# armando-palacio/opticomlib

Hardware: AMD Instinct MI355X
Metric: SSFM sample*steps/sec, 2^20-sample dual-pol fiber (higher is better)
Workload: dtype c64

## Files before the change

### opticomlib_amd/csrc/ssfm_host.hip

```cpp
#include <hip/hip_runtime.h>

#include <algorithm>
#include <memory>
#include <cmath>
#include <cstdarg>
#include <cstddef>
#include <cstdio>
#include <cstdlib>
#include <chrono>
#include <cstring>
#include <atomic>
#include <condition_variable>
#include <functional>
#include <mutex>
#include <new>
#include <string>
#include <thread>
#include <type_traits>
#include <vector>

#include "ssfm_amd.h"
#include "ssfm_common.hpp"
#include "ssfm_kernels.hpp"
#include "ssfm_launch.hpp"
// ... 687 lines not shown
            lanes_from_pool = true;
            ++g_lane_pairs_reused;
        }
        if (!lane_stream[0]) HIP_TRY(hipStreamCreateWithPriority(lane_stream[0].out(), hipStreamNonBlocking, prio_hi));
        stream = lane_stream[0];
        for (Event* e : {&ev0, &ev1}) HIP_TRY(hipEventCreate(e->out()));
        if (const char* e = std::getenv("SSFM_LANE_THREADS")) lane_threads = std::atoi(e) != 0;
        HIP_TRY(hipEventCreateWithFlags(fork_ev.out(), hipEventDisableTiming));
        for (int g = 1; g < nlanes; ++g) {
            if (!(lanes_from_pool && g == 1)) HIP_TRY(hipStreamCreateWithPriority(lane_stream[g].out(), hipStreamNonBlocking, prio_hi));
            HIP_TRY(hipEventCreateWithFlags(lane_ev[g].out(), hipEventDisableTiming));
        }
        lanes_active = nlanes;
        return SSFM_OK;
    }
    int make_tables() {
        HIP_TRY(F_own.reserve(cb * n * batch));
        HIP_TRY(P_own.reserve(sizeof(T) * n * batch));
        F = F_own; P = P_own;
        Y = F;
        if (u16) { HIP_TRY(Y_own.reserve(cb * n * batch)); Y = Y_own; }
        if (u16 || sizeof(T) == 8) {
            const long long nA = (long long)(N1 / E) * N2, nB = (long long)E * N2;
            HIP_TRY(twA.reserve(cb * nA));
            HIP_TRY(twB.reserve(cb * nB));
            const int C_ = cols_per_tile<T>();
            hipLaunchKernelGGL(k_make_tw_tiles<T>, dim3((unsigned)((nA + 255) / 256)), dim3(256), 0, stream, twA.get(), N1 / E, 1ll, N2, C_, (long long)n, (int)u16, N2 / Ef);
            hipLaunchKernelGGL(k_make_tw_tiles<T>, dim3((unsigned)((nB + 255) / 256)), dim3(256), 0, stream, twB.get(), E, (long long)(N1 / E), N2, C_, (long long)n, (int)u16, N2 / Ef);
        } else {
            HIP_TRY(twN.reserve(cb * n));
            hipLaunchKernelGGL(k_make_twN<T>, dim3((unsigned)((n + 255) / 256)), dim3(256), 0, stream, twN.get(), N1, N2, cols_per_tile<T>(), E, (int)u16, N2 / Ef);
        }
        if (int rc = make_line_table(&tw1, N1, E)) return rc;
        if (int rc = make_line_table(&tw2, N2, Ef)) return rc;
        HIP_TRY(dnat.reserve(cb * n_full));
        HIP_TRY(dperm.reserve(cb * n));
        return SSFM_OK;
    }
    int make_split_extras() {
        HIP_TRY(Fnat.reserve(cb * n_full * batch_full));
        HIP_TRY(hipMemsetAsync(Fnat, 0, cb * n_full * batch_full, stream));
        HIP_TRY(split_twA.reserve(sizeof(double2) * (size_t)split_R * N1));
        HIP_TRY(split_twB.reserve(sizeof(double2) * (size_t)split_R * N2));
        const long long nt = (long long)split_R * (N1 + N2);
        hipLaunchKernelGGL(k_make_split_twiddles, dim3((unsigned)((nt + 255) / 256)), dim3(256), 0, stream, split_twA.get(), split_twB.get(), N1, N2, split_R);
        HIP_TRY(hipGetLastError());
        return SSFM_OK;
    }
    int make_engine_extras() {
        if (Ef_fly != Ef) {
            if (int rc = make_line_table(&tw2_fly, N2, Ef_fly)) return rc;
            HIP_TRY(dperm_fly.reserve(cb * n));
        }
        if (const char* e = std::getenv("SSFM_ADAPT_FUSED")) fused_ok = std::atoi(e) != 0;
        if (const char* e = std::getenv("SSFM_MEDIUM")) medium_ok = std::atoi(e) != 0;
        if (const char* e = std::getenv("SSFM_MEDIUM_ADAPT")) medium_adapt_ok = std::atoi(e) != 0;
        if (const char* e = std::getenv("SSFM_MEDIUM_SPLIT")) medium_split_ok = std::atoi(e) != 0;
        if (const char* e = std::getenv("SSFM_FUSED_PATIENCE_TICKS")) medium_patience = std::atoll(e);
        if (const char* e = std::getenv("SSFM_PHASE_TABLE")) phase_tables = std::atoi(e) != 0;
        if (const char* e = std::getenv("SSFM_FORCE_FLY")) force_fly = std::atoi(e) != 0;
        if (sizeof(T) == 4 && medium_shape(N1, N2) && (medium_ok || medium_adapt_ok)) (void)pick_xcc();
        if (small) {
            if (int rc = make_line_table(&tw_small, (int)n, small_points<T>((int)n))) return rc;
            HIP_TRY(dsmall.reserve(cb * n));
        }
        HIP_TRY(st.reserve(sizeof(AdaptState<T>)));
        HIP_TRY(hipMemsetAsync(P, 0, sizeof(T) * n * batch, stream));
        HIP_TRY(hipGetLastError());
        HIP_TRY(hipStreamSynchronize(stream));
        return SSFM_OK;
    }
    int rate_lanes_at_creation() {
        for (Event* e : {&lane_e0, &lane_e1, &run_e0, &run_e1}) HIP_TRY(hipEventCreate(e->out()));
        HIP_TRY(hipMemsetAsync(F, 0, cb * n * batch, stream));
        if (Y != F) HIP_TRY(hipMemsetAsync(Y, 0, cb * n * batch, stream));
        HIP_TRY(hipMemsetAsync(dperm, 0, cb * n, stream));
        if (dperm_fly) HIP_TRY(hipMemsetAsync(dperm_fly, 0, cb * n, stream));
        bool replaced = false;
        if (lanes_from_pool && nlanes == 2) lanes_ok = true;
        else {
            ++g_lane_ratings;
            if (int rc = rate_and_replace_lanes(F, Y, P, &replaced)) return rc;
        }
        if (!lanes_ok) lane_strikes = 1;
// ... 124 lines not shown
        else lane_suspect = 0;
        return SSFM_OK;
    }
    int heal_lanes() {
        ++lane_heals;
        HIP_TRY(hipStreamSynchronize(stream));
        const size_t cb = sizeof(cx<T>) * (size_t)n * batch;
        DeviceBuffer<cx<T>> Fx_own, Yx_own;
        DeviceBuffer<T> Px_own;
        if (Fx_own.reserve(cb) != hipSuccess) { (void)hipGetLastError(); return SSFM_OK; }
        if (Y != F && Yx_own.reserve(cb) != hipSuccess) { (void)hipGetLastError(); return SSFM_OK; }
        if (Px_own.reserve(sizeof(T) * (size_t)n * batch) != hipSuccess) { (void)hipGetLastError(); return SSFM_OK; }
        cx<T>* const Fx = Fx_own; cx<T>* const Yx = Y != F ? Yx_own.get() : Fx; T* const Px = Px_own;
        (void)hipMemsetAsync(Fx, 0, cb, stream);
        if (Yx != Fx) (void)hipMemsetAsync(Yx, 0, cb, stream);
        (void)hipMemsetAsync(Px, 0, sizeof(T) * (size_t)n * batch, stream);
        const float seen = lane_pair_us;
        bool replaced = false;
        const int rc = rate_and_replace_lanes(Fx, Yx, Px, &replaced);
        (void)hipStreamSynchronize(stream);
        if (rc != SSFM_OK) return rc;
        if (replaced) ++lanes_remade;
        if (lanes_ok) {
            lane_strikes = 0;
            if (!replaced) lane_pair_us = lane_last_us;
            else if (seen > 0.f && seen < lane_pair_us) lane_pair_us = seen;
        } else if (++lane_strikes >= 2) {
            lanes_active = 1;
            lanes_dropped = 1;
        }
        return SSFM_OK;
    }

    int make_line_table(DeviceBuffer<cx<T>>* out, int L, int E) {
        const int M = fft_nstages(L, E);
        const int total = fft_tw_entries(L, E, (int)sizeof(T));
        std::vector<cx<T>> tab((size_t)(total > 0 ? total : 1));
        for (int S = 1; S < M; ++S) {
            const int R = fft_radix(L, S, E), NB = E / R, KU = fft_tw_ku(L, S, E), off = fft_tw_offset(L, S, E, (int)sizeof(T));
            for (int i = 0; i < NB; ++i)
                for (int u = 1; u < R; ++u)
                    for (int ku = 0; ku < KU; ++ku) {
                        const int q = fft_tw_exponent(L, E, S, i, u, ku) % L;
                        const double ang = -2.0 * 3.14159265358979323846 * (double)q / (double)L;
                        cx<T> w; w.x = (T)std::cos(ang); w.y = (T)std::sin(ang);
                        if (q == 0) { w.x = (T)1; w.y = (T)0; }
                        if (4 * q == L) { w.x = (T)0; w.y = (T)-1; }
                        if (2 * q == L) { w.x = (T)-1; w.y = (T)0; }
                        if (4 * q == 3 * L) { w.x = (T)0; w.y = (T)1; }
                        tab[(size_t)off + (size_t)fft_tw_index(L, S, E, (int)sizeof(T), i * (R - 1) + (u - 1), ku)] = w;
                    }
        }
        HIP_TRY(out->reserve(sizeof(cx<T>) * tab.size()));
        HIP_TRY(hipMemcpy(out->get(), tab.data(), sizeof(cx<T>) * tab.size(), hipMemcpyHostToDevice));
        return SSFM_OK;
    }

#if SSFM_TRACE
    DeviceBuffer<unsigned long long> trace_buf;
    int trace_cap = 0; std::atomic<int> trace_next{0};
    std::vector<int> trace_kind;
    int trace_begin(int launches) {
        if (!std::getenv("SSFM_TRACE_FILE")) return SSFM_OK;
        if (trace_cap < launches) {
            HIP_TRY(trace_buf.reserve(sizeof(unsigned long long) * 1024 * launches));
            trace_cap = launches;
        }
        HIP_TRY(hipMemset(trace_buf, 0, sizeof(unsigned long long) * 1024 * launches));
        trace_next = 0;
        trace_kind.assign(launches, 0);
        return SSFM_OK;
    }
    template <typename A> void trace_tag(A& a, int kind, int lane) {
        a.trace = nullptr; a.trace_slot = 0;
        if (trace_buf) { const int slot = trace_next.fetch_add(1); if (slot < trace_cap) { a.trace = trace_buf; a.trace_slot = slot; trace_kind[slot] = kind * 16 + lane; } }
    }
    int trace_dump() {
        const char* path = std::getenv("SSFM_TRACE_FILE");
        if (!path || !trace_buf) return SSFM_OK;
        HIP_TRY(hipStreamSynchronize(stream));
        const int nt = std::min((int)trace_next, trace_cap);
        std::vector<unsigned long long> raw(1024 * (size_t)nt), h(4 * (size_t)nt);
        HIP_TRY(hipMemcpy(raw.data(), trace_buf, sizeof(unsigned long long) * raw.size(), hipMemcpyDeviceToHost));
        for (int i = 0; i < nt; ++i) {
            unsigned long long fs = ~0ull, ls = 0, fe = ~0ull, le = 0;
// ... 1816 lines not shown
```

### opticomlib_amd/csrc/ssfm_kernels.hpp

```cpp
#pragma once
#include "ssfm_route.hpp"
#include "wgfft.hpp"

#ifndef SSFM_ABLATE
#define SSFM_ABLATE 0
#endif
#define SSFM_ABL_NO_TWN ((SSFM_ABLATE & 1) != 0)
#define SSFM_ABL_NO_P ((SSFM_ABLATE & 2) != 0)
#define SSFM_ABL_NO_TAB ((SSFM_ABLATE & 4) != 0)
#define SSFM_ABL_NO_FFT ((SSFM_ABLATE & 8) != 0)
#define SSFM_ABL_NO_NL ((SSFM_ABLATE & 16) != 0)

template <typename T, bool U16> __host__ __device__ constexpr bool stream_policy() { return U16; }
template <typename T, bool U16> __host__ __device__ constexpr bool twn_compute() { return U16 || sizeof(T) == 8; }

#ifndef SSFM_TRACE
#define SSFM_TRACE 0
#endif
#if SSFM_TRACE
#define SSFM_TRACE_ARGS unsigned long long* trace; int trace_slot;
#define SSFM_TRACE_BEGIN(a)                                                                     \
    if ((a).trace && threadIdx.x == 0) {                                                        \
        unsigned hw_, xc_;                                                                      \
        asm volatile("s_getreg_b32 %0, hwreg(HW_REG_HW_ID)" : "=s"(hw_));                       \
// ... 1142 lines not shown
        const double e = flat ? e0 : exp_acc<double>(m[t].x * h);
        m[t] = mk<double>((e * cs) * inv_n, (e * sn) * inv_n);
    }
}

template <typename T, int N2, int ROWS, int E, int MODE, bool U16, bool PK = false, bool H = false>
__device__ __forceinline__ void freq_body(const FreqArgs<T>& a, const unsigned bid) {
    static_assert(!H || (sizeof(T) == 8 && !U16 && !PK && MODE == FM_TABLE), "H (see time_body): the plain layout of a complex128 plan, a table of complex numbers");
    constexpr int Q = N2 / E;
    extern __shared__ __attribute__((aligned(16))) unsigned char smem_raw[];
    cx<T>* lds = reinterpret_cast<cx<T>*>(smem_raw);

    T h = a.h;
    constexpr bool FLY = MODE == FM_FLY || MODE == FM_FLY_IM;
    SSFM_TRACE_BEGIN(a);
    const int tid = threadIdx.x;
    const int j = tid % Q;
    const int rr = tid / Q;
    int kgrp, brow;
    xcd_unit_row(bid, a.N1 / ROWS, a.rows, kgrp, brow);
    const int k1 = kgrp * ROWS + rr;
    const long long row = (long long)brow * a.N1 + k1;
    cx<T>* __restrict__ Frow = a.F + row * N2;
    const cx<T>* __restrict__ trow = a.tab + (MODE == FM_TABLE_ROWS ? row : (long long)k1) * N2;
    using RI = RowIdx<row_pad_shift(E)>;
    const RI idx{rr * row_lds_elems(N2, E)};

    cx<T> v[E];
    cx<T> m[E];
    LineTw<T, N2, E> tw;
    SSFM_STAMP(0);
    typedef T u4_t __attribute__((ext_vector_type(4)));
    constexpr bool EARLY_PHASE = MODE == FM_PHASE;
    TwStaged<T, N2, E, ROWS * N2 / E> tws;
    line_twiddles_prefetch<T, N2, E, ROWS * N2 / E>(tws, a.tw2, tid);
    unsigned pu[E];
    double pt[sizeof(T) == 8 ? E : 1];
    auto load_phases = [&]() {
        if constexpr (sizeof(T) == 8) {
            typedef double d2_t __attribute__((ext_vector_type(2)));
            const d2_t* __restrict__ P2 = reinterpret_cast<const d2_t*>(reinterpret_cast<const double*>(a.tab) + (long long)k1 * N2) + j;
#pragma unroll
            for (int g = 0; g < E / 2; ++g) {
                const d2_t q = P2[g * Q];
                pt[2 * g] = q.x; pt[2 * g + 1] = q.y;
            }
        } else {
        typedef unsigned u32x4 __attribute__((ext_vector_type(4)));
        const u32x4* __restrict__ P4 = reinterpret_cast<const u32x4*>(reinterpret_cast<const unsigned*>(a.tab) + (long long)k1 * N2) + j;
#pragma unroll
        for (int g = 0; g < E / 4; ++g) {
            u32x4 q;
            if (SSFM_ABL_NO_TAB) q = 0x12345678u; else q = P4[g * Q];
            pu[4 * g] = q.x; pu[4 * g + 1] = q.y; pu[4 * g + 2] = q.z; pu[4 * g + 3] = q.w;
        }
        }
    };
    auto phase_factors = [&]() {
#pragma unroll
        for (int t = 0; t < E; ++t) {
            if constexpr (sizeof(T) == 8) m[t] = phase64_factor(pt[t], a.amp);
            else m[t] = phase32_factor(pu[t], a.amp);
        }
    };
    constexpr bool EARLY_FLY = FLY;
    auto load_table = [&]() {
        if constexpr (MODE == FM_FLY_IM) {
// ... 16 lines not shown
            m[2 * g] = mk<T>(q.x, q.y);
            m[2 * g + 1] = mk<T>(q.z, q.w);
        }
    };
    if constexpr (EARLY_PHASE) load_phases();
    if constexpr (EARLY_FLY) load_table();
    constexpr bool INV_ONLY = MODE == FM_INV_ONLY;
    if (U16 && (!INV_ONLY || a.u16 == 2)) {
        if constexpr (PK && sizeof(T) == 4) {
            const __amdgpu_buffer_rsrc_t rs = __builtin_amdgcn_make_buffer_rsrc((void*)Frow, 0, N2 * (int)sizeof(cx<T>), 0x00020000);
#pragma unroll
            for (int g = 0; g < E / 2; ++g) {
                const u32x4_t q = load16_sc1(rs, (g * Q + j) * 16);
                v[2 * g] = mk<T>(__uint_as_float(q.x), __uint_as_float(q.y));
                v[2 * g + 1] = mk<T>(__uint_as_float(q.z), __uint_as_float(q.w));
            }
        } else {
#pragma unroll
        for (int g = 0; g < E / 2; ++g) {
            const u4_t q = stream_load<true>(reinterpret_cast<const u4_t*>(Frow) + g * Q + j);
            v[2 * g] = mk<T>(q.x, q.y);
            v[2 * g + 1] = mk<T>(q.z, q.w);
        }
        }
    } else if constexpr (H) {
        const cx<float>* __restrict__ F32 = reinterpret_cast<const cx<float>*>(a.F) + row * N2;
#pragma unroll
        for (int t = 0; t < E; ++t) { const cx<float> q = F32[j + t * Q]; v[t] = mk<T>((T)q.x, (T)q.y); }
    } else {
#pragma unroll
        for (int t = 0; t < E; ++t) v[t] = Frow[j + t * Q];
    }
    cx<T>* ldsT = lds + (fft_nstages(N2, E) > 1 ? ROWS * row_lds_elems(N2, E) : 0);
    line_twiddles_issue_regs<T, N2, E>(tw, j, a.tw2);
    if constexpr (MODE == FM_TABLE || MODE == FM_TABLE_ROWS) load_table();
    if ((FLY || MODE == FM_FWD_ONLY || MODE == FM_INV_ONLY) && a.st != nullptr) {
        const StepState<T> S = a.st->cur[a.step & 1];
        if (S.done || a.st->error != 0u) return;
        h = S.h;
    }
    SSFM_STAMP(1);
#if SSFM_STAMPS
    asm volatile("s_waitcnt vmcnt(0)" ::: "memory");
    SSFM_STAMP(2);
#endif
    line_twiddles_commit<T, N2, E, ROWS * N2 / E>(tws, ldsT, tid);
    auto fly = [&]() {
        T ph[E];
#pragma unroll
        for (int t = 0; t < E; ++t) ph[t] = m[t].y * h;
        bool flat = true;
#pragma unroll
        for (int t = 1; t < E; ++t) flat = flat && (m[t].x == m[0].x);
        const T e0 = exp_acc<T>(m[0].x * h);
        fly_factors<E>(m, ph, flat, e0, h, a.inv_n);
    };
    if constexpr (EARLY_PHASE) {
        phase_factors();
        __builtin_amdgcn_sched_barrier(0);
    }
    if constexpr (EARLY_FLY) {
        fly();
        __builtin_amdgcn_sched_barrier(0);
    }
    if (fft_tw_lds_entries(N2, E) > 0) __syncthreads();
    line_twiddles_fetch<T, N2, E>(tw, j, ldsT);
    if (!SSFM_ABL_NO_FFT && !INV_ONLY) fft_line<T, N2, E, -1, 0, RI>(v, lds, 0, j, idx, tw);
    if (MODE == FM_FWD_ONLY) {
        if (U16 && a.u16 == 2) {
#pragma unroll
            for (int g = 0; g < E / 2; ++g) {
                u4_t q;
                q.x = v[2 * g].x; q.y = v[2 * g].y; q.z = v[2 * g + 1].x; q.w = v[2 * g + 1].y;
                pass_store<PK>(reinterpret_cast<u4_t*>(Frow) + g * Q + j, q);
            }
            return;
        }
#pragma unroll
        for (int t = 0; t < E; ++t) pass_store<PK>(&Frow[j + t * Q], v[t]);
        return;
    }
    SSFM_STAMP(3);
    if constexpr (!INV_ONLY) {
#pragma unroll
    for (int t = 0; t < E; ++t) v[t] = cmul(v[t], m[t]);
    }
    SSFM_STAMP(4);
    if (!SSFM_ABL_NO_FFT) fft_line<T, N2, E, +1, (fft_nstages(N2, E) == 1 ? 0 : 1), RI>(v, lds, 0, j, idx, tw);
    SSFM_STAMP(5);
    if (U16) {
#pragma unroll
        for (int g = 0; g < E / 2; ++g) {
            u4_t q;
            q.x = v[2 * g].x; q.y = v[2 * g].y; q.z = v[2 * g + 1].x; q.w = v[2 * g + 1].y;
            pass_store<PK>(reinterpret_cast<u4_t*>(Frow) + g * Q + j, q);
        }
    } else if constexpr (H) {
        cx<float>* __restrict__ F32 = reinterpret_cast<cx<float>*>(a.F) + row * N2;
#pragma unroll
// ... 12 lines not shown
    SSFM_TRACE_END(a);
}

template <typename T, int N2, int ROWS, int E, int MODE, bool U16 = false>
__global__ SSFM_KERNEL_BOUNDS(ROWS * N2 / E, sizeof(T), E) void k_freq(cx<T>* F, const cx<T>* tab, const cx<T>* tw2, const AdaptState<T>* st, T h, T amp, T inv_n, int step, int N1,
                                                                     int rows, int u16
#if SSFM_TRACE
                                                                     , unsigned long long* trace, int trace_slot
#endif
                                                                     ) {
    FreqArgs<T> a;
    a.F = F; a.tab = tab; a.tw2 = tw2; a.st = st; a.h = h; a.amp = amp; a.inv_n = inv_n; a.step = step; a.N1 = N1; a.rows = rows; a.u16 = u16;
#if SSFM_TRACE
    a.trace = trace; a.trace_slot = trace_slot;
#endif
    freq_body<T, N2, ROWS, E, MODE, U16, false>(a, blockIdx.x);
}
template <typename T, int N2, int ROWS, int E, int MODE>
__global__ SSFM_KERNEL_BOUNDS(ROWS * N2 / E, sizeof(T), E) void k_freq_h(cx<T>* F, const cx<T>* tab, const cx<T>* tw2, const AdaptState<T>* st, T h, T amp, T inv_n, int step, int N1,
                                                                       int rows, int u16, const int* done
#if SSFM_TRACE
                                                                       , unsigned long long* trace, int trace_slot
#endif
                                                                       ) {
    if (done != nullptr && *done) return;
    FreqArgs<T> a;
    a.F = F; a.tab = tab; a.tw2 = tw2; a.st = st; a.h = h; a.amp = amp; a.inv_n = inv_n; a.step = step; a.N1 = N1; a.rows = rows; a.u16 = u16;
#if SSFM_TRACE
    a.trace = trace; a.trace_slot = trace_slot;
#endif
    freq_body<T, N2, ROWS, E, MODE, false, false, true>(a, blockIdx.x);
}
template <typename T, int N2, int ROWS, int E, int MODE, bool U16 = false>
__global__ __launch_bounds__(ROWS * N2 / E) void k_freq_half(cx<T>* F, const cx<T>* tab, const cx<T>* tw2, const AdaptState<T>* st, T h, T amp, T inv_n, int step, int N1,
                                                            int rows, int u16
#if SSFM_TRACE
                                                            , unsigned long long* trace, int trace_slot
#endif
                                                            ) {
    static_assert(MODE == FM_FWD_ONLY || MODE == FM_INV_ONLY, "k_freq_half: the transform-only modes");
    FreqArgs<T> a;
    a.F = F; a.tab = tab; a.tw2 = tw2; a.st = st; a.h = h; a.amp = amp; a.inv_n = inv_n; a.step = step; a.N1 = N1; a.rows = rows; a.u16 = u16;
#if SSFM_TRACE
    a.trace = trace; a.trace_slot = trace_slot;
#endif
    freq_body<T, N2, ROWS, E, MODE, U16, false>(a, blockIdx.x);
}
#if SSFM_TRACE
#define SSFM_FREQ_KERNEL_ARGS(a) (a).F, (a).tab, (a).tw2, (a).st, (a).h, (a).amp, (a).inv_n, (a).step, (a).N1, (a).rows, (a).u16, (a).trace, (a).trace_slot
#else
#define SSFM_FREQ_KERNEL_ARGS(a) (a).F, (a).tab, (a).tw2, (a).st, (a).h, (a).amp, (a).inv_n, (a).step, (a).N1, (a).rows, (a).u16
#endif

constexpr int kSmallTabs = 4;
template <typename T> struct MediumArgs {
    cx<T>* F;
    cx<T>* Y;
    T* P;
    const cx<T>* twA;
    const cx<T>* twB;
    const cx<T>* tw1;
    const cx<T>* tw2;
    const cx<T>* tab[kSmallTabs];
    T amp[kSmallTabs];
    const T* hs;
    const unsigned char* which;
    unsigned long long* bar;
// ... 958 lines not shown
```

### opticomlib_amd/csrc/ssfm_launch.hpp

```cpp
#pragma once
#include <hip/hip_runtime.h>

#include <cstddef>

#include "ssfm_kernels.hpp"

namespace ssfm {
template <typename T> constexpr size_t col_pass_lds(int N1, int C, int E) {
    return ((fft_nstages(N1, E) > 1 ? (size_t)N1 * C : 0) + (size_t)E * C + (size_t)fft_tw_lds_entries(N1, E)) * sizeof(cx<T>);
}
template <typename T> constexpr size_t row_pass_lds(int N, int E, int ROWS, size_t extra = 0) {
    return ((fft_nstages(N, E) > 1 ? (size_t)ROWS * row_lds_elems(N, E) : 0) + (size_t)fft_tw_lds_entries(N, E) + extra) * sizeof(cx<T>);
}

template <auto Kernel, size_t LDS, typename... Args>
hipError_t launch_kernel(dim3 grid, dim3 block, hipStream_t s, const Args&... args) {
    if constexpr (LDS > 48 * 1024) {
        static const hipError_t raised = hipFuncSetAttribute(reinterpret_cast<const void*>(Kernel), hipFuncAttributeMaxDynamicSharedMemorySize, (int)LDS);
        if (raised != hipSuccess) return raised;
    }
    hipLaunchKernelGGL(Kernel, grid, block, LDS, s, args...);
    return hipGetLastError();
}
}
```

### opticomlib_amd/csrc/wgfft.hpp

```cpp
#pragma once
#include <hip/hip_runtime.h>

#ifndef SSFM_STAMPS
#define SSFM_STAMPS 0
#endif
#if SSFM_STAMPS
extern __device__ unsigned long long* g_stamp_buf;
#define SSFM_STAMP(i)                                                                         \
    do {                                                                                      \
        __builtin_amdgcn_sched_barrier(0);                                                    \
        if (threadIdx.x == 0) {                                                               \
            unsigned long long t_;                                                            \
            asm volatile("s_memtime %0\n\ts_waitcnt lgkmcnt(0)" : "=s"(t_)::"memory");         \
            g_stamp_buf[blockIdx.x * 16 + (i)] = t_;                                          \
        }                                                                                     \
        __builtin_amdgcn_sched_barrier(0);                                                    \
    } while (0)
#else
#define SSFM_STAMP(i) do { } while (0)
#endif


namespace ssfm {

typedef float  cf32 __attribute__((ext_vector_type(2)));
typedef double cf64 __attribute__((ext_vector_type(2)));
template <typename T> struct cx_of;
template <> struct cx_of<float>  { using type = cf32; };
template <> struct cx_of<double> { using type = cf64; };
template <typename T> using cx = typename cx_of<T>::type;
template <typename C> struct real_of;
template <> struct real_of<cf32> { using type = float; };
template <> struct real_of<cf64> { using type = double; };

// ... 98 lines not shown
        x[0] = cadd(e0, o0); x[4] = csub(e0, o0);
        x[1] = cadd(e1, o1); x[5] = csub(e1, o1);
        x[2] = add_rot<DIR>(e2, o2); x[6] = sub_rot<DIR>(e2, o2);
        x[3] = cadd(e3, o3); x[7] = csub(e3, o3);
    }
};
template <> struct Dft<16> {
    template <int DIR, typename C> static __device__ __forceinline__ void run(C* x) {
        using T = typename real_of<C>::type;
        using K = RadixConst<T>;
#pragma unroll
        for (int b = 0; b < 4; ++b) dft4<DIR>(x[b], x[b + 4], x[b + 8], x[b + 12]);
        x[1 + 4]  = cmuld<DIR>(x[1 + 4], mk<T>(K::cA, -K::sA));
        x[1 + 8]  = mul_w8_1<DIR, 1>(x[1 + 8]);
        x[1 + 12] = cmuld<DIR>(x[1 + 12], mk<T>(K::sB, -K::cB));
        x[2 + 4]  = mul_w8_1<DIR, 0>(x[2 + 4]);
        x[2 + 8]  = rot90<DIR>(x[2 + 8]);
        x[2 + 12] = mul_w8_3<DIR, 1>(x[2 + 12]);
        x[3 + 4]  = cmuld<DIR>(x[3 + 4], mk<T>(K::sB, -K::cB));
        x[3 + 8]  = mul_w8_3<DIR, 0>(x[3 + 8]);
        x[3 + 12] = cmuld<DIR>(x[3 + 12], mk<T>(-K::cB, K::sB));
        C y[16];
#pragma unroll
        for (int q = 0; q < 4; ++q) {
            C a = x[4 * q], b = x[4 * q + 1], c = x[4 * q + 2], d = x[4 * q + 3];
            dft4<DIR>(a, b, c, d);
            y[q] = a; y[q + 4] = b; y[q + 8] = c; y[q + 12] = d;
        }
#pragma unroll
        for (int i = 0; i < 16; ++i) x[i] = y[i];
    }
};

__host__ __device__ constexpr int ilog2(int v) { return v <= 1 ? 0 : 1 + ilog2(v >> 1); }
__host__ __device__ constexpr int fft_nstages(int L, int E) {
    return E == 16 ? (L <= 16 ? 1 : (L <= 256 ? 2 : (L <= 4096 ? 3 : 4))) : (ilog2(L) + 2) / 3;
}
__host__ __device__ constexpr int fft_radix(int L, int s, int E) {
    return E == 16 ? (L == 16   ? 16
                    : L == 32   ? (s == 0 ? 8 : 4)
                    : L == 64   ? 8
                    : L == 128  ? (s == 0 ? 16 : 8)
                    : L == 256  ? 16
                    : L == 512  ? 8
                    : L == 1024 ? (s == 0 ? 16 : 8)
                    : L == 2048 ? (s <= 1 ? 16 : 8)
                    : L == 4096 ? 16
                    :             (s <= 2 ? 16 : 2))
                   : (s < ilog2(L) / 3 ? 8 : (1 << (ilog2(L) % 3)));
}
__host__ __device__ constexpr int fft_ls(int L, int s, int E) {
    return s == 0 ? 1 : fft_ls(L, s - 1, E) * fft_radix(L, s - 1, E);
}

template <typename T, int E, int L = 0> __host__ __device__ constexpr bool tw_lazy() {
    return sizeof(T) == 8 && E == 16;
}

template <typename T, int L, int E, bool LAZY = tw_lazy<T, E, L>()> struct LineTw {
    static constexpr int M = fft_nstages(L, E);
    cx<T> w[M > 1 ? M - 1 : 1][E - 1];
};
template <typename T, int L, int E> struct LineTw<T, L, E, true> {
    static constexpr int M = fft_nstages(L, E);
    const cx<T>* g[M > 1 ? M - 1 : 1];
    const cx<T>* l[M > 1 ? M - 1 : 1];
};
__host__ __device__ constexpr int fft_tw_slots_of(int L, int S, int E) { return (E / fft_radix(L, S, E)) * (fft_radix(L, S, E) - 1); }
__host__ __device__ constexpr int fft_tw_ku(int L, int S, int E) { return fft_ls(L, S, E) < L / E ? fft_ls(L, S, E) : L / E; }
__host__ __device__ constexpr bool fft_tw_via_lds(int L, int S, int E) { return fft_tw_slots_of(L, S, E) * fft_tw_ku(L, S, E) <= 512; }
__host__ __device__ constexpr bool fft_tw_paired(int L, int S, int E, int ts) {
    return ts == 4 && !fft_tw_via_lds(L, S, E);
}
__host__ __device__ constexpr int fft_tw_stage_entries(int L, int S, int E, int ts) {
    return fft_tw_paired(L, S, E, ts) ? ((fft_tw_slots_of(L, S, E) + 1) / 2) * 2 * fft_tw_ku(L, S, E)
                                      : ((fft_tw_slots_of(L, S, E) * fft_tw_ku(L, S, E) + 1) / 2) * 2;
}
__host__ __device__ constexpr int fft_tw_offset(int L, int S, int E, int ts) {
    return S <= 1 ? 0 : fft_tw_offset(L, S - 1, E, ts) + fft_tw_stage_entries(L, S - 1, E, ts);
}
__host__ __device__ constexpr int fft_tw_entries(int L, int E, int ts) { return fft_tw_offset(L, fft_nstages(L, E), E, ts); }
__host__ __device__ constexpr int fft_tw_index(int L, int S, int E, int ts, int slot, int ku) {
    return fft_tw_paired(L, S, E, ts) ? ((slot >> 1) * fft_tw_ku(L, S, E) + ku) * 2 + (slot & 1) : slot * fft_tw_ku(L, S, E) + ku;
}
__host__ __device__ constexpr int fft_tw_lds_offset(int L, int S, int E) {
    return S <= 1 ? 0 : fft_tw_lds_offset(L, S - 1, E) + (fft_tw_via_lds(L, S - 1, E) ? fft_tw_slots_of(L, S - 1, E) * fft_tw_ku(L, S - 1, E) : 0);
}
__host__ __device__ constexpr int fft_tw_lds_entries(int L, int E) { return fft_tw_lds_offset(L, fft_nstages(L, E), E); }
__host__ __device__ constexpr int fft_tw_exponent(int L, int E, int S, int i, int u, int ku) {
    return ((ku + i * (L / E)) & (fft_ls(L, S, E) - 1)) * u * (L / (fft_ls(L, S, E) * fft_radix(L, S, E)));
}

template <typename T, int L, int E, int S>
__device__ __forceinline__ void tw_stage_issue(LineTw<T, L, E>& tw, const int j, const cx<T>* __restrict__ tab, cx<T>* ldsT,
                                               const int tid, const int nthreads) {
    constexpr int SLOTS = fft_tw_slots_of(L, S, E);
    constexpr int KU = fft_tw_ku(L, S, E);
    constexpr int OFF = fft_tw_offset(L, S, E, (int)sizeof(T));
    if constexpr (fft_tw_paired(L, S, E, (int)sizeof(T))) {
        typedef T w4_t __attribute__((ext_vector_type(4)));
        const w4_t* __restrict__ p4 = reinterpret_cast<const w4_t*>(tab + OFF) + (j & (KU - 1));
#pragma unroll
        for (int pr = 0; pr < (SLOTS + 1) / 2; ++pr) {
            const w4_t q = p4[pr * KU];
            tw.w[S - 1][2 * pr] = mk<T>(q.x, q.y);
            if (2 * pr + 1 < SLOTS) tw.w[S - 1][2 * pr + 1] = mk<T>(q.z, q.w);
        }
    } else if constexpr (fft_tw_via_lds(L, S, E)) {
        constexpr int LOFF = fft_tw_lds_offset(L, S, E);
        for (int e = tid; e < SLOTS * KU; e += nthreads) ldsT[LOFF + e] = tab[OFF + e];
    } else if constexpr (tw_lazy<T, E, L>()) {
        tw.g[S - 1] = tab + OFF + (j & (KU - 1));
    } else {
#pragma unroll
        for (int sl = 0; sl < SLOTS; ++sl) tw.w[S - 1][sl] = tab[OFF + sl * KU + (j & (KU - 1))];
    }
}
template <typename T, int L, int E, int S>
__device__ __forceinline__ void tw_stage_fetch(LineTw<T, L, E>& tw, const int j, const cx<T>* ldsT) {
    if constexpr (fft_tw_via_lds(L, S, E)) {
        constexpr int SLOTS = fft_tw_slots_of(L, S, E);
        constexpr int KU = fft_tw_ku(L, S, E);
        constexpr int LOFF = fft_tw_lds_offset(L, S, E);
        if constexpr (tw_lazy<T, E, L>()) {
            tw.l[S - 1] = ldsT + LOFF + (j & (KU - 1));
        } else {
#pragma unroll
            for (int sl = 0; sl < SLOTS; ++sl) tw.w[S - 1][sl] = ldsT[LOFF + sl * KU + (j & (KU - 1))];
        }
    }
}
template <typename T, int L, int E, int S>
__device__ __forceinline__ cx<T> tw_get(const LineTw<T, L, E>& tw, const int slot) {
    if constexpr (tw_lazy<T, E, L>()) {
        constexpr int KU = fft_tw_ku(L, S, E);
        if constexpr (fft_tw_via_lds(L, S, E)) return tw.l[S - 1][slot * KU];
        else return tw.g[S - 1][slot * KU];
    } else {
        return tw.w[S - 1][slot];
    }
}
template <typename T, int L, int E>
__device__ __forceinline__ void line_twiddles_issue(LineTw<T, L, E>& tw, const int j, const cx<T>* __restrict__ tab, cx<T>* ldsT,
                                                    const int tid, const int nthreads) {
    constexpr int M = fft_nstages(L, E);
    if constexpr (M > 1) tw_stage_issue<T, L, E, 1>(tw, j, tab, ldsT, tid, nthreads);
    if constexpr (M > 2) tw_stage_issue<T, L, E, 2>(tw, j, tab, ldsT, tid, nthreads);
    if constexpr (M > 3) tw_stage_issue<T, L, E, 3>(tw, j, tab, ldsT, tid, nthreads);
}
__host__ __device__ constexpr int fft_tw_prefetch_count(int L, int E, int NT, int S = 1) {
    return S >= fft_nstages(L, E) ? 0
         : (fft_tw_via_lds(L, S, E) ? (fft_tw_slots_of(L, S, E) * fft_tw_ku(L, S, E) + NT - 1) / NT : 0) + fft_tw_prefetch_count(L, E, NT, S + 1);
}
template <typename T, int L, int E, int NT> struct TwStaged {
    static constexpr int PF = fft_tw_prefetch_count(L, E, NT);
    cx<T> r[PF > 0 ? PF : 1];
};
template <typename T, int L, int E, int NT, int S>
__device__ __forceinline__ void tw_stage_prefetch(TwStaged<T, L, E, NT>& p, int& k, const cx<T>* __restrict__ tab, const int tid) {
    if constexpr (fft_tw_via_lds(L, S, E)) {
        constexpr int NS = fft_tw_slots_of(L, S, E) * fft_tw_ku(L, S, E), OFF = fft_tw_offset(L, S, E, (int)sizeof(T));
#pragma unroll
        for (int i = 0; i * NT < NS; ++i) {
            const int e = tid + i * NT;
            p.r[k++] = e < NS ? tab[OFF + e] : mk<T>((T)0, (T)0);
        }
    }
}
template <typename T, int L, int E, int NT, int S>
__device__ __forceinline__ void tw_stage_commit(const TwStaged<T, L, E, NT>& p, int& k, cx<T>* ldsT, const int tid) {
    if constexpr (fft_tw_via_lds(L, S, E)) {
        constexpr int NS = fft_tw_slots_of(L, S, E) * fft_tw_ku(L, S, E), LOFF = fft_tw_lds_offset(L, S, E);
#pragma unroll
        for (int i = 0; i * NT < NS; ++i) {
            const int e = tid + i * NT;
            if (e < NS) ldsT[LOFF + e] = p.r[k];
            ++k;
        }
    }
}
template <typename T, int L, int E, int NT>
__device__ __forceinline__ void line_twiddles_prefetch(TwStaged<T, L, E, NT>& p, const cx<T>* __restrict__ tab, const int tid) {
    constexpr int M = fft_nstages(L, E);
    int k = 0;
    if constexpr (M > 1) tw_stage_prefetch<T, L, E, NT, 1>(p, k, tab, tid);
    if constexpr (M > 2) tw_stage_prefetch<T, L, E, NT, 2>(p, k, tab, tid);
    if constexpr (M > 3) tw_stage_prefetch<T, L, E, NT, 3>(p, k, tab, tid);
}
template <typename T, int L, int E, int NT>
__device__ __forceinline__ void line_twiddles_commit(const TwStaged<T, L, E, NT>& p, cx<T>* ldsT, const int tid) {
    constexpr int M = fft_nstages(L, E);
    int k = 0;
    if constexpr (M > 1) tw_stage_commit<T, L, E, NT, 1>(p, k, ldsT, tid);
    if constexpr (M > 2) tw_stage_commit<T, L, E, NT, 2>(p, k, ldsT, tid);
    if constexpr (M > 3) tw_stage_commit<T, L, E, NT, 3>(p, k, ldsT, tid);
}
template <typename T, int L, int E>
__device__ __forceinline__ void line_twiddles_issue_regs(LineTw<T, L, E>& tw, const int j, const cx<T>* __restrict__ tab) {
    constexpr int M = fft_nstages(L, E);
    if constexpr (M > 1 && !fft_tw_via_lds(L, 1, E)) tw_stage_issue<T, L, E, 1>(tw, j, tab, nullptr, 0, 1);
    if constexpr (M > 2 && !fft_tw_via_lds(L, 2, E)) tw_stage_issue<T, L, E, 2>(tw, j, tab, nullptr, 0, 1);
    if constexpr (M > 3 && !fft_tw_via_lds(L, 3, E)) tw_stage_issue<T, L, E, 3>(tw, j, tab, nullptr, 0, 1);
}
template <typename T, int L, int E>
__device__ __forceinline__ void line_twiddles_fetch(LineTw<T, L, E>& tw, const int j, const cx<T>* ldsT) {
    constexpr int M = fft_nstages(L, E);
    if constexpr (M > 1) tw_stage_fetch<T, L, E, 1>(tw, j, ldsT);
    if constexpr (M > 2) tw_stage_fetch<T, L, E, 2>(tw, j, ldsT);
    if constexpr (M > 3) tw_stage_fetch<T, L, E, 3>(tw, j, ldsT);
}

template <typename T, int L, int E, int DIR, int S, int XP, typename IDX>
__device__ __forceinline__ void fft_stage(cx<T> (&v)[E], cx<T>* lds, const int BUF, const int j, const IDX& idx,
                                          const LineTw<T, L, E>& tw) {
    constexpr int M  = fft_nstages(L, E);
    constexpr int R  = fft_radix(L, S, E);
    constexpr int NB = E / R;
    constexpr int Q  = L / E;
    constexpr int LS = fft_ls(L, S, E);

#ifdef SSFM_STAMP_FFT
    if (DIR < 0) SSFM_STAMP_FFT(7 + 3 * S);
#endif
    if constexpr (S > 0) {
        const cx<T>* src = lds + ((XP + S - 1) & 1) * BUF;
#pragma unroll
        for (int i = 0; i < NB; ++i) {
            const int jb = j + i * Q;
#pragma unroll
            for (int u = 0; u < R; ++u) v[i + u * NB] = src[idx(jb + u * (L / R))];
        }
#pragma unroll
        for (int i = 0; i < NB; ++i) {
#pragma unroll
            for (int u = 1; u < R; ++u)
                v[i + u * NB] = cmuld<DIR>(v[i + u * NB], tw_get<T, L, E, S>(tw, i * (R - 1) + (u - 1)));
        }
    }
#ifdef SSFM_STAMP_FFT
    if (DIR < 0) SSFM_STAMP_FFT(8 + 3 * S);
#endif
#pragma unroll
// ... 49 lines not shown
```

Baseline: 68.34 billion.

## Replace large per-stage row-FFT twiddle tables with a compact quarter-wave table in LDS

For fp32 row FFT stages whose twiddles were too large for LDS and were loaded per thread from global memory, the table now stores only the first quarter of the unit circle. The kernel stages it into the row exchange buffer, gathers entries from LDS, and rebuilds the full twiddle with sign and swap bit tricks. This removes per-thread global twiddle loads in the frequency kernel. The cost is extra barriers, bit manipulation and LDS sizing constraints, plus a waves-per-EU occupancy hint on k_freq_half. Table generation code moves into a shared plan header.

```diff
diff --git a/opticomlib_amd/csrc/fft_plan.hpp b/opticomlib_amd/csrc/fft_plan.hpp
--- /dev/null
+++ b/opticomlib_amd/csrc/fft_plan.hpp
@@ -0,0 +1,106 @@
+#pragma once
+#include <cmath>
+#include <cstddef>
+#include <vector>
+
+#if defined(__HIPCC__)
+#define SSFM_HD __host__ __device__
+#define SSFM_HD_INLINE __host__ __device__ __forceinline__
+#else
+#define SSFM_HD
+#define SSFM_HD_INLINE inline
+#endif
+
+namespace ssfm {
+
+SSFM_HD constexpr int ilog2(int v) { return v <= 1 ? 0 : 1 + ilog2(v >> 1); }
+SSFM_HD constexpr int fft_nstages(int L, int E) {
+    return E == 16 ? (L <= 16 ? 1 : (L <= 256 ? 2 : (L <= 4096 ? 3 : 4))) : (ilog2(L) + 2) / 3;
+}
+SSFM_HD constexpr int fft_radix(int L, int s, int E) {
+    return E == 16 ? (L == 16   ? 16
+                    : L == 32   ? (s == 0 ? 8 : 4)
+                    : L == 64   ? 8
+                    : L == 128  ? (s == 0 ? 16 : 8)
+                    : L == 256  ? 16
+                    : L == 512  ? 8
+                    : L == 1024 ? (s == 0 ? 16 : 8)
+                    : L == 2048 ? (s <= 1 ? 16 : 8)
+                    : L == 4096 ? 16
+                    :             (s <= 2 ? 16 : 2))
+                   : (s < ilog2(L) / 3 ? 8 : (1 << (ilog2(L) % 3)));
+}
+SSFM_HD constexpr int fft_ls(int L, int s, int E) {
+    return s == 0 ? 1 : fft_ls(L, s - 1, E) * fft_radix(L, s - 1, E);
+}
+
+SSFM_HD constexpr int fft_tw_slots_of(int L, int S, int E) { return (E / fft_radix(L, S, E)) * (fft_radix(L, S, E) - 1); }
+SSFM_HD constexpr int fft_tw_ku(int L, int S, int E) { return fft_ls(L, S, E) < L / E ? fft_ls(L, S, E) : L / E; }
+SSFM_HD constexpr bool fft_tw_via_lds(int L, int S, int E) { return fft_tw_slots_of(L, S, E) * fft_tw_ku(L, S, E) <= 512; }
+SSFM_HD constexpr bool fft_tw_paired(int L, int S, int E, int ts) {
+    return ts == 4 && !fft_tw_via_lds(L, S, E);
+}
+SSFM_HD constexpr int fft_tw_stage_entries(int L, int S, int E, int ts) {
+    return fft_tw_paired(L, S, E, ts) ? ((fft_tw_slots_of(L, S, E) + 1) / 2) * 2 * fft_tw_ku(L, S, E)
+                                      : ((fft_tw_slots_of(L, S, E) * fft_tw_ku(L, S, E) + 1) / 2) * 2;
+}
+SSFM_HD constexpr int fft_tw_offset(int L, int S, int E, int ts) {
+    return S <= 1 ? 0 : fft_tw_offset(L, S - 1, E, ts) + fft_tw_stage_entries(L, S - 1, E, ts);
+}
+SSFM_HD constexpr int fft_tw_entries(int L, int E, int ts) { return fft_tw_offset(L, fft_nstages(L, E), E, ts); }
+SSFM_HD constexpr int fft_tw_index(int L, int S, int E, int ts, int slot, int ku) {
+    return fft_tw_paired(L, S, E, ts) ? ((slot >> 1) * fft_tw_ku(L, S, E) + ku) * 2 + (slot & 1) : slot * fft_tw_ku(L, S, E) + ku;
+}
+SSFM_HD constexpr int fft_tw_lds_offset(int L, int S, int E) {
+    return S <= 1 ? 0 : fft_tw_lds_offset(L, S - 1, E) + (fft_tw_via_lds(L, S - 1, E) ? fft_tw_slots_of(L, S - 1, E) * fft_tw_ku(L, S - 1, E) : 0);
+}
+SSFM_HD constexpr int fft_tw_lds_entries(int L, int E) { return fft_tw_lds_offset(L, fft_nstages(L, E), E); }
+SSFM_HD constexpr int fft_tw_exponent(int L, int E, int S, int i, int u, int ku) {
+    return ((ku + i * (L / E)) & (fft_ls(L, S, E) - 1)) * u * (L / (fft_ls(L, S, E) * fft_radix(L, S, E)));
+}
+
+SSFM_HD constexpr bool fft_tw_compact(int L, int S, int E, int ts) { return ts == 4 && !fft_tw_via_lds(L, S, E); }
+SSFM_HD constexpr int fft_tw_first_compact(int L, int E, int ts, int S = 1) {
+    return S >= fft_nstages(L, E) ? fft_nstages(L, E) : (fft_tw_compact(L, S, E, ts) ? S : fft_tw_first_compact(L, E, ts, S + 1));
+}
+SSFM_HD constexpr bool fft_tw_has_compact(int L, int E, int ts) { return fft_tw_first_compact(L, E, ts) < fft_nstages(L, E); }
+SSFM_HD constexpr int fft_tw_base_offset(int L, int E, int ts) { return fft_tw_offset(L, fft_tw_first_compact(L, E, ts), E, ts); }
+SSFM_HD constexpr int fft_tw_compact_entries(int L, int E, int ts) { return fft_tw_base_offset(L, E, ts) + L / 4; }
+SSFM_HD constexpr int fft_tw_base_pos(int r) { return r; }
+SSFM_HD constexpr int fft_tw_base_lds(int L) { return fft_tw_base_pos(L / 4 - 1) + 1; }
+template <int L> SSFM_HD_INLINE void fft_tw_rebuild(unsigned& x, unsigned& y, const unsigned q) {
+    constexpr int SH = 31 - ilog2(L / 2);
+    const bool swap = (q & (unsigned)(L / 4)) != 0u;
+    const unsigned a = swap ? y : x, b = swap ? x : y;
+    x = a ^ ((q & (unsigned)(L / 2)) << SH);
+    y = b ^ (((q + (unsigned)(L / 4)) & (unsigned)(L / 2)) << SH);
+}
+
+template <typename C, typename T> inline C fft_twiddle(int q, int L) {
+    const double ang = -2.0 * 3.14159265358979323846 * (double)q / (double)L;
+    C w; w.x = (T)std::cos(ang); w.y = (T)std::sin(ang);
+    if (q == 0) { w.x = (T)1; w.y = (T)0; }
+    if (4 * q == L) { w.x = (T)0; w.y = (T)-1; }
+    if (2 * q == L) { w.x = (T)-1; w.y = (T)0; }
+    if (4 * q == 3 * L) { w.x = (T)0; w.y = (T)1; }
+    return w;
+}
+template <typename C, typename T> inline std::vector<C> fft_line_table(int L, int E, bool compact) {
+    const int ts = (int)sizeof(T), M = fft_nstages(L, E);
+    compact = compact && fft_tw_has_compact(L, E, ts);
+    const int last = compact ? fft_tw_first_compact(L, E, ts) : M;
+    const int total = compact ? fft_tw_compact_entries(L, E, ts) : fft_tw_entries(L, E, ts);
+    std::vector<C> tab((size_t)(total > 0 ? total : 1));
+    for (int S = 1; S < last; ++S) {
+        const int R = fft_radix(L, S, E), NB = E / R, KU = fft_tw_ku(L, S, E), off = fft_tw_offset(L, S, E, ts);
+        for (int i = 0; i < NB; ++i)
+            for (int u = 1; u < R; ++u)
+                for (int ku = 0; ku < KU; ++ku)
+                    tab[(size_t)off + (size_t)fft_tw_index(L, S, E, ts, i * (R - 1) + (u - 1), ku)] = fft_twiddle<C, T>(fft_tw_exponent(L, E, S, i, u, ku) % L, L);
+    }
+    if (compact)
+        for (int r = 0; r < L / 4; ++r) tab[(size_t)fft_tw_base_offset(L, E, ts) + (size_t)r] = fft_twiddle<C, T>(r, L);
+    return tab;
+}
+
+}
diff --git a/opticomlib_amd/csrc/ssfm_host.hip b/opticomlib_amd/csrc/ssfm_host.hip
--- a/opticomlib_amd/csrc/ssfm_host.hip
+++ b/opticomlib_amd/csrc/ssfm_host.hip
@@ -743,7 +743,7 @@
             hipLaunchKernelGGL(k_make_twN<T>, dim3((unsigned)((n + 255) / 256)), dim3(256), 0, stream, twN.get(), N1, N2, cols_per_tile<T>(), E, (int)u16, N2 / Ef);
         }
         if (int rc = make_line_table(&tw1, N1, E)) return rc;
-        if (int rc = make_line_table(&tw2, N2, Ef)) return rc;
+        if (int rc = make_line_table(&tw2, N2, Ef, true)) return rc;
         HIP_TRY(dnat.reserve(cb * n_full));
         HIP_TRY(dperm.reserve(cb * n));
         return SSFM_OK;
@@ -760,7 +760,7 @@
     }
     int make_engine_extras() {
         if (Ef_fly != Ef) {
-            if (int rc = make_line_table(&tw2_fly, N2, Ef_fly)) return rc;
+            if (int rc = make_line_table(&tw2_fly, N2, Ef_fly, true)) return rc;
             HIP_TRY(dperm_fly.reserve(cb * n));
         }
         if (const char* e = std::getenv("SSFM_ADAPT_FUSED")) fused_ok = std::atoi(e) != 0;
@@ -951,25 +951,8 @@
         return SSFM_OK;
     }
 
-    int make_line_table(DeviceBuffer<cx<T>>* out, int L, int E) {
-        const int M = fft_nstages(L, E);
-        const int total = fft_tw_entries(L, E, (int)sizeof(T));
-        std::vector<cx<T>> tab((size_t)(total > 0 ? total : 1));
-        for (int S = 1; S < M; ++S) {
-            const int R = fft_radix(L, S, E), NB = E / R, KU = fft_tw_ku(L, S, E), off = fft_tw_offset(L, S, E, (int)sizeof(T));
-            for (int i = 0; i < NB; ++i)
-                for (int u = 1; u < R; ++u)
-                    for (int ku = 0; ku < KU; ++ku) {
-                        const int q = fft_tw_exponent(L, E, S, i, u, ku) % L;
-                        const double ang = -2.0 * 3.14159265358979323846 * (double)q / (double)L;
-                        cx<T> w; w.x = (T)std::cos(ang); w.y = (T)std::sin(ang);
-                        if (q == 0) { w.x = (T)1; w.y = (T)0; }
-                        if (4 * q == L) { w.x = (T)0; w.y = (T)-1; }
-                        if (2 * q == L) { w.x = (T)-1; w.y = (T)0; }
-                        if (4 * q == 3 * L) { w.x = (T)0; w.y = (T)1; }
-                        tab[(size_t)off + (size_t)fft_tw_index(L, S, E, (int)sizeof(T), i * (R - 1) + (u - 1), ku)] = w;
-                    }
-        }
+    int make_line_table(DeviceBuffer<cx<T>>* out, int L, int E, bool compact = false) {
+        const std::vector<cx<T>> tab = fft_line_table<cx<T>, T>(L, E, compact);
         HIP_TRY(out->reserve(sizeof(cx<T>) * tab.size()));
         HIP_TRY(hipMemcpy(out->get(), tab.data(), sizeof(cx<T>) * tab.size(), hipMemcpyHostToDevice));
         return SSFM_OK;
diff --git a/opticomlib_amd/csrc/ssfm_kernels.hpp b/opticomlib_amd/csrc/ssfm_kernels.hpp
--- a/opticomlib_amd/csrc/ssfm_kernels.hpp
+++ b/opticomlib_amd/csrc/ssfm_kernels.hpp
@@ -1198,7 +1198,10 @@
     SSFM_STAMP(0);
     typedef T u4_t __attribute__((ext_vector_type(4)));
     constexpr bool EARLY_PHASE = MODE == FM_PHASE;
-    TwStaged<T, N2, E, ROWS * N2 / E> tws;
+    constexpr bool COMPACT = fft_tw_has_compact(N2, E, (int)sizeof(T));
+    static_assert(!COMPACT || (ROWS == 1 && !PK && fft_tw_base_lds(N2) <= row_lds_elems(N2, E)),
+                  "the quarter table borrows the exchange buffer of a launch's only row pass: one row, no earlier pass of the same workgroup still reading it");
+    TwStaged<T, N2, E, ROWS * N2 / E, COMPACT> tws;
     line_twiddles_prefetch<T, N2, E, ROWS * N2 / E>(tws, a.tw2, tid);
     unsigned pu[E];
     double pt[sizeof(T) == 8 ? E : 1];
@@ -1281,7 +1284,7 @@
         for (int t = 0; t < E; ++t) v[t] = Frow[j + t * Q];
     }
     cx<T>* ldsT = lds + (fft_nstages(N2, E) > 1 ? ROWS * row_lds_elems(N2, E) : 0);
-    line_twiddles_issue_regs<T, N2, E>(tw, j, a.tw2);
+    if constexpr (!COMPACT) line_twiddles_issue_regs<T, N2, E>(tw, j, a.tw2);
     if constexpr (MODE == FM_TABLE || MODE == FM_TABLE_ROWS) load_table();
     if ((FLY || MODE == FM_FWD_ONLY || MODE == FM_INV_ONLY) && a.st != nullptr) {
         const StepState<T> S = a.st->cur[a.step & 1];
@@ -1293,7 +1296,7 @@
     asm volatile("s_waitcnt vmcnt(0)" ::: "memory");
     SSFM_STAMP(2);
 #endif
-    line_twiddles_commit<T, N2, E, ROWS * N2 / E>(tws, ldsT, tid);
+    line_twiddles_commit<T, N2, E, ROWS * N2 / E>(tws, ldsT, tid, lds);
     auto fly = [&]() {
         T ph[E];
 #pragma unroll
@@ -1304,6 +1307,11 @@
         const T e0 = exp_acc<T>(m[0].x * h);
         fly_factors<E>(m, ph, flat, e0, h, a.inv_n);
     };
+    if constexpr (COMPACT) {
+        __syncthreads();
+        line_twiddles_fetch<T, N2, E>(tw, j, ldsT);
+        line_twiddles_gather<T, N2, E>(tw, j, lds);
+    }
     if constexpr (EARLY_PHASE) {
         phase_factors();
         __builtin_amdgcn_sched_barrier(0);
@@ -1312,8 +1320,13 @@
         fly();
         __builtin_amdgcn_sched_barrier(0);
     }
-    if (fft_tw_lds_entries(N2, E) > 0) __syncthreads();
-    line_twiddles_fetch<T, N2, E>(tw, j, ldsT);
+    if constexpr (COMPACT) {
+        __syncthreads();
+        line_twiddles_rebuild<T, N2, E>(tw, j);
+    } else {
+        if (fft_tw_lds_entries(N2, E) > 0) __syncthreads();
+        line_twiddles_fetch<T, N2, E>(tw, j, ldsT);
+    }
     if (!SSFM_ABL_NO_FFT && !INV_ONLY) fft_line<T, N2, E, -1, 0, RI>(v, lds, 0, j, idx, tw);
     if (MODE == FM_FWD_ONLY) {
         if (U16 && a.u16 == 2) {
@@ -1392,7 +1405,7 @@
     freq_body<T, N2, ROWS, E, MODE, false, false, true>(a, blockIdx.x);
 }
 template <typename T, int N2, int ROWS, int E, int MODE, bool U16 = false>
-__global__ __launch_bounds__(ROWS * N2 / E) void k_freq_half(cx<T>* F, const cx<T>* tab, const cx<T>* tw2, const AdaptState<T>* st, T h, T amp, T inv_n, int step, int N1,
+__global__ __launch_bounds__(ROWS * N2 / E) __attribute__((amdgpu_waves_per_eu(ROWS * N2 / E >= 512 ? 4 : 1))) void k_freq_half(cx<T>* F, const cx<T>* tab, const cx<T>* tw2, const AdaptState<T>* st, T h, T amp, T inv_n, int step, int N1,
                                                             int rows, int u16
 #if SSFM_TRACE
                                                             , unsigned long long* trace, int trace_slot
diff --git a/opticomlib_amd/csrc/ssfm_launch.hpp b/opticomlib_amd/csrc/ssfm_launch.hpp
--- a/opticomlib_amd/csrc/ssfm_launch.hpp
+++ b/opticomlib_amd/csrc/ssfm_launch.hpp
@@ -10,7 +10,9 @@
     return ((fft_nstages(N1, E) > 1 ? (size_t)N1 * C : 0) + (size_t)E * C + (size_t)fft_tw_lds_entries(N1, E)) * sizeof(cx<T>);
 }
 template <typename T> constexpr size_t row_pass_lds(int N, int E, int ROWS, size_t extra = 0) {
-    return ((fft_nstages(N, E) > 1 ? (size_t)ROWS * row_lds_elems(N, E) : 0) + (size_t)fft_tw_lds_entries(N, E) + extra) * sizeof(cx<T>);
+    const size_t rows = fft_nstages(N, E) > 1 ? (size_t)ROWS * row_lds_elems(N, E) : 0;
+    const size_t base = fft_tw_has_compact(N, E, (int)sizeof(T)) ? (size_t)fft_tw_base_lds(N) : 0;
+    return ((rows > base ? rows : base) + (size_t)fft_tw_lds_entries(N, E) + extra) * sizeof(cx<T>);
 }
 
 template <auto Kernel, size_t LDS, typename... Args>
diff --git a/opticomlib_amd/csrc/wgfft.hpp b/opticomlib_amd/csrc/wgfft.hpp
--- a/opticomlib_amd/csrc/wgfft.hpp
+++ b/opticomlib_amd/csrc/wgfft.hpp
@@ -1,5 +1,7 @@
 #pragma once
 #include <hip/hip_runtime.h>
+
+#include "fft_plan.hpp"
 
 #ifndef SSFM_STAMPS
 #define SSFM_STAMPS 0
@@ -164,27 +166,6 @@
     }
 };
 
-__host__ __device__ constexpr int ilog2(int v) { return v <= 1 ? 0 : 1 + ilog2(v >> 1); }
-__host__ __device__ constexpr int fft_nstages(int L, int E) {
-    return E == 16 ? (L <= 16 ? 1 : (L <= 256 ? 2 : (L <= 4096 ? 3 : 4))) : (ilog2(L) + 2) / 3;
-}
-__host__ __device__ constexpr int fft_radix(int L, int s, int E) {
-    return E == 16 ? (L == 16   ? 16
-                    : L == 32   ? (s == 0 ? 8 : 4)
-                    : L == 64   ? 8
-                    : L == 128  ? (s == 0 ? 16 : 8)
-                    : L == 256  ? 16
-                    : L == 512  ? 8
-                    : L == 1024 ? (s == 0 ? 16 : 8)
-                    : L == 2048 ? (s <= 1 ? 16 : 8)
-                    : L == 4096 ? 16
-                    :             (s <= 2 ? 16 : 2))
-                   : (s < ilog2(L) / 3 ? 8 : (1 << (ilog2(L) % 3)));
-}
-__host__ __device__ constexpr int fft_ls(int L, int s, int E) {
-    return s == 0 ? 1 : fft_ls(L, s - 1, E) * fft_radix(L, s - 1, E);
-}
-
 template <typename T, int E, int L = 0> __host__ __device__ constexpr bool tw_lazy() {
     return sizeof(T) == 8 && E == 16;
 }
@@ -198,31 +179,6 @@
     const cx<T>* g[M > 1 ? M - 1 : 1];
     const cx<T>* l[M > 1 ? M - 1 : 1];
 };
-__host__ __device__ constexpr int fft_tw_slots_of(int L, int S, int E) { return (E / fft_radix(L, S, E)) * (fft_radix(L, S, E) - 1); }
-__host__ __device__ constexpr int fft_tw_ku(int L, int S, int E) { return fft_ls(L, S, E) < L / E ? fft_ls(L, S, E) : L / E; }
-__host__ __device__ constexpr bool fft_tw_via_lds(int L, int S, int E) { return fft_tw_slots_of(L, S, E) * fft_tw_ku(L, S, E) <= 512; }
-__host__ __device__ constexpr bool fft_tw_paired(int L, int S, int E, int ts) {
-    return ts == 4 && !fft_tw_via_lds(L, S, E);
-}
-__host__ __device__ constexpr int fft_tw_stage_entries(int L, int S, int E, int ts) {
-    return fft_tw_paired(L, S, E, ts) ? ((fft_tw_slots_of(L, S, E) + 1) / 2) * 2 * fft_tw_ku(L, S, E)
-                                      : ((fft_tw_slots_of(L, S, E) * fft_tw_ku(L, S, E) + 1) / 2) * 2;
-}
-__host__ __device__ constexpr int fft_tw_offset(int L, int S, int E, int ts) {
-    return S <= 1 ? 0 : fft_tw_offset(L, S - 1, E, ts) + fft_tw_stage_entries(L, S - 1, E, ts);
-}
-__host__ __device__ constexpr int fft_tw_entries(int L, int E, int ts) { return fft_tw_offset(L, fft_nstages(L, E), E, ts); }
-__host__ __device__ constexpr int fft_tw_index(int L, int S, int E, int ts, int slot, int ku) {
-    return fft_tw_paired(L, S, E, ts) ? ((slot >> 1) * fft_tw_ku(L, S, E) + ku) * 2 + (slot & 1) : slot * fft_tw_ku(L, S, E) + ku;
-}
-__host__ __device__ constexpr int fft_tw_lds_offset(int L, int S, int E) {
-    return S <= 1 ? 0 : fft_tw_lds_offset(L, S - 1, E) + (fft_tw_via_lds(L, S - 1, E) ? fft_tw_slots_of(L, S - 1, E) * fft_tw_ku(L, S - 1, E) : 0);
-}
-__host__ __device__ constexpr int fft_tw_lds_entries(int L, int E) { return fft_tw_lds_offset(L, fft_nstages(L, E), E); }
-__host__ __device__ constexpr int fft_tw_exponent(int L, int E, int S, int i, int u, int ku) {
-    return ((ku + i * (L / E)) & (fft_ls(L, S, E) - 1)) * u * (L / (fft_ls(L, S, E) * fft_radix(L, S, E)));
-}
-
 template <typename T, int L, int E, int S>
 __device__ __forceinline__ void tw_stage_issue(LineTw<T, L, E>& tw, const int j, const cx<T>* __restrict__ tab, cx<T>* ldsT,
                                                const int tid, const int nthreads) {
@@ -284,12 +240,16 @@
     return S >= fft_nstages(L, E) ? 0
          : (fft_tw_via_lds(L, S, E) ? (fft_tw_slots_of(L, S, E) * fft_tw_ku(L, S, E) + NT - 1) / NT : 0) + fft_tw_prefetch_count(L, E, NT, S + 1);
 }
-template <typename T, int L, int E, int NT> struct TwStaged {
+__host__ __device__ constexpr int fft_tw_base_loads(int L, int NT) { return (L / 8 + NT - 1) / NT; }
+template <typename T, int L, int E, int NT, bool BASE = false> struct TwStaged {
     static constexpr int PF = fft_tw_prefetch_count(L, E, NT);
+    static constexpr int PB = BASE && fft_tw_has_compact(L, E, (int)sizeof(T)) ? fft_tw_base_loads(L, NT) : 0;
+    typedef T w4_t __attribute__((ext_vector_type(4)));
     cx<T> r[PF > 0 ? PF : 1];
-};
-template <typename T, int L, int E, int NT, int S>
-__device__ __forceinline__ void tw_stage_prefetch(TwStaged<T, L, E, NT>& p, int& k, const cx<T>* __restrict__ tab, const int tid) {
+    w4_t b[PB > 0 ? PB : 1];
+};
+template <typename T, int L, int E, int NT, int S, bool BASE>
+__device__ __forceinline__ void tw_stage_prefetch(TwStaged<T, L, E, NT, BASE>& p, int& k, const cx<T>* __restrict__ tab, const int tid) {
     if constexpr (fft_tw_via_lds(L, S, E)) {
         constexpr int NS = fft_tw_slots_of(L, S, E) * fft_tw_ku(L, S, E), OFF = fft_tw_offset(L, S, E, (int)sizeof(T));
 #pragma unroll
@@ -299,8 +259,8 @@
         }
     }
 }
-template <typename T, int L, int E, int NT, int S>
-__device__ __forceinline__ void tw_stage_commit(const TwStaged<T, L, E, NT>& p, int& k, cx<T>* ldsT, const int tid) {
+template <typename T, int L, int E, int NT, int S, bool BASE>
+__device__ __forceinline__ void tw_stage_commit(const TwStaged<T, L, E, NT, BASE>& p, int& k, cx<T>* ldsT, const int tid) {
     if constexpr (fft_tw_via_lds(L, S, E)) {
         constexpr int NS = fft_tw_slots_of(L, S, E) * fft_tw_ku(L, S, E), LOFF = fft_tw_lds_offset(L, S, E);
 #pragma unroll
@@ -311,21 +271,39 @@
         }
     }
 }
-template <typename T, int L, int E, int NT>
-__device__ __forceinline__ void line_twiddles_prefetch(TwStaged<T, L, E, NT>& p, const cx<T>* __restrict__ tab, const int tid) {
+template <typename T, int L, int E, int NT, bool BASE>
+__device__ __forceinline__ void line_twiddles_prefetch(TwStaged<T, L, E, NT, BASE>& p, const cx<T>* __restrict__ tab, const int tid) {
     constexpr int M = fft_nstages(L, E);
     int k = 0;
     if constexpr (M > 1) tw_stage_prefetch<T, L, E, NT, 1>(p, k, tab, tid);
     if constexpr (M > 2) tw_stage_prefetch<T, L, E, NT, 2>(p, k, tab, tid);
     if constexpr (M > 3) tw_stage_prefetch<T, L, E, NT, 3>(p, k, tab, tid);
-}
-template <typename T, int L, int E, int NT>
-__device__ __forceinline__ void line_twiddles_commit(const TwStaged<T, L, E, NT>& p, cx<T>* ldsT, const int tid) {
+    constexpr int PB = TwStaged<T, L, E, NT, BASE>::PB;
+    if constexpr (PB > 0) {
+        static_assert((L / 8) % NT == 0, "every thread loads the same number of entry pairs");
+        typedef T w4_t __attribute__((ext_vector_type(4)));
+        constexpr int BOFF = fft_tw_base_offset(L, E, (int)sizeof(T));
+        const w4_t* __restrict__ b4 = reinterpret_cast<const w4_t*>(tab + BOFF) + tid;
+#pragma unroll
+        for (int i = 0; i < PB; ++i) p.b[i] = b4[i * NT];
+    }
+}
+template <typename T, int L, int E, int NT, bool BASE>
+__device__ __forceinline__ void line_twiddles_commit(const TwStaged<T, L, E, NT, BASE>& p, cx<T>* ldsT, const int tid, cx<T>* ldsB = nullptr) {
     constexpr int M = fft_nstages(L, E);
     int k = 0;
     if constexpr (M > 1) tw_stage_commit<T, L, E, NT, 1>(p, k, ldsT, tid);
     if constexpr (M > 2) tw_stage_commit<T, L, E, NT, 2>(p, k, ldsT, tid);
     if constexpr (M > 3) tw_stage_commit<T, L, E, NT, 3>(p, k, ldsT, tid);
+    constexpr int PB = TwStaged<T, L, E, NT, BASE>::PB;
+    if constexpr (PB > 0) {
+#pragma unroll
+        for (int i = 0; i < PB; ++i) {
+            const int r = 2 * (tid + i * NT);
+            ldsB[fft_tw_base_pos(r)] = mk<T>(p.b[i].x, p.b[i].y);
+            ldsB[fft_tw_base_pos(r) + 1] = mk<T>(p.b[i].z, p.b[i].w);
+        }
+    }
 }
 template <typename T, int L, int E>
 __device__ __forceinline__ void line_twiddles_issue_regs(LineTw<T, L, E>& tw, const int j, const cx<T>* __restrict__ tab) {
@@ -340,6 +318,44 @@
     if constexpr (M > 1) tw_stage_fetch<T, L, E, 1>(tw, j, ldsT);
     if constexpr (M > 2) tw_stage_fetch<T, L, E, 2>(tw, j, ldsT);
     if constexpr (M > 3) tw_stage_fetch<T, L, E, 3>(tw, j, ldsT);
+}
+template <typename T, int L, int E, int S, bool REBUILD>
+__device__ __forceinline__ void tw_stage_compact(LineTw<T, L, E>& tw, const int j, const cx<T>* ldsB) {
+    if constexpr (fft_tw_compact(L, S, E, (int)sizeof(T))) {
+        constexpr int R = fft_radix(L, S, E), NB = E / R, Q = L / E, LS = fft_ls(L, S, E), STEP = L / (LS * R);
+#pragma unroll
+        for (int i = 0; i < NB; ++i) {
+            const unsigned k = (unsigned)(j + i * Q) & (unsigned)(LS - 1);
+#pragma unroll
+            for (int u = 1; u < R; ++u) {
+                const unsigned q = k * (unsigned)(u * STEP);
+                cx<T>& w = tw.w[S - 1][i * (R - 1) + (u - 1)];
+                if constexpr (!REBUILD) {
+                    static_assert(fft_tw_base_pos(L / 4 - 1) == L / 4 - 1, "the table is not padded (fft_plan.hpp)");
+                    const unsigned off = (k * (unsigned)sizeof(cx<T>)) * (unsigned)(u * STEP) & (unsigned)((L / 4 - 1) * sizeof(cx<T>));
+                    w = *reinterpret_cast<const cx<T>*>(reinterpret_cast<const char*>(ldsB) + off);
+                } else {
+                    unsigned x = __float_as_uint(w.x), y = __float_as_uint(w.y);
+                    fft_tw_rebuild<L>(x, y, q);
+                    w = mk<T>(__uint_as_float(x), __uint_as_float(y));
+                }
+            }
+        }
+    }
+}
+template <typename T, int L, int E>
+__device__ __forceinline__ void line_twiddles_gather(LineTw<T, L, E>& tw, const int j, const cx<T>* ldsB) {
+    constexpr int M = fft_nstages(L, E);
+    if constexpr (M > 1) tw_stage_compact<T, L, E, 1, false>(tw, j, ldsB);
+    if constexpr (M > 2) tw_stage_compact<T, L, E, 2, false>(tw, j, ldsB);
+    if constexpr (M > 3) tw_stage_compact<T, L, E, 3, false>(tw, j, ldsB);
+}
+template <typename T, int L, int E>
+__device__ __forceinline__ void line_twiddles_rebuild(LineTw<T, L, E>& tw, const int j) {
+    constexpr int M = fft_nstages(L, E);
+    if constexpr (M > 1) tw_stage_compact<T, L, E, 1, true>(tw, j, nullptr);
+    if constexpr (M > 2) tw_stage_compact<T, L, E, 2, true>(tw, j, nullptr);
+    if constexpr (M > 3) tw_stage_compact<T, L, E, 3, true>(tw, j, nullptr);
 }
 
 template <typename T, int L, int E, int DIR, int S, int XP, typename IDX>
```

Result: no change. 67.97 billion (-0.5%).
